# plus-rkwitt/flooder

Measured on AMD Instinct MI355X. Metric: M points×simplices/s (coverage sweep), higher is better.
Workload: dtype f32; 1 GPU; 1M-point 3D Gaussian, 1k landmarks, points_per_edge 30, max_dimension 3, fp32 coverage sweep (BASELINE.json configs[1]); points=1000000, landmarks=1000, top_simplices=6052, top_simplices_rank0=6052, swept_dimension=3, method=cell, parallelism=single GPU

## Files before the change

flooder_amd/_native.py:

```python

from __future__ import annotations

import ctypes
import os
from ctypes import c_char_p, c_float, c_int, c_int32, c_int64, c_uint32, c_void_p

_PKG_DIR = os.path.dirname(os.path.abspath(__file__))
LIB_PATH = os.environ.get("FLOODER_HIP_LIB") or os.path.join(_PKG_DIR, "libflooder_hip.so")



class _Block(ctypes.Structure):

    ABI = 1

    def __init__(self, **fields):
        super().__init__()
        self.size = ctypes.sizeof(self)
        self.abi = self.ABI
        known = {name for name, _ in self._fields_}
        for key, value in fields.items():
            if key not in known:
                raise TypeError(f"{type(self).__name__} has no field {key!r}")
            if value is not None and not isinstance(value, (int, float)):
                value = ptr(value)
            setattr(self, key, value)


def _fields(spec: str):
    kinds = {"p": c_void_p, "i64": c_int64, "i32": c_int32, "u32": c_uint32, "f32": c_float}
    out = []
    for item in spec.replace("\n", " ").split(";"):
        item = item.strip()
        if item:
            kind, name = item.split()
            out.append((name, kinds[kind]))
    return out


class FusedSweep(_Block):

    _fields_ = _fields("""u32 size; u32 abi; p pts_sorted; i64 n_pts; i32 dim; i32 k1; p nodes; p density_grid; p cloud_box;
        p verts; p weights; i32 R; i32 n_faces; i64 n_simplices; p memb; f32 alpha; i32 n_coarse; p coarse_rows; p parents;
        p face_bits; p face_slot; p d2_scratch; p flag_list; p flag_count; p flag_key; p flag_hist; p flag_sorted; p top;
        p top_list; p top_count; p simplex_weight; p plane_scratch; p wit_queue; p wit_item_list; p wit_stats;
        p cell_queue; p defer_list; p defer_c; p defer_ctl; p light_list; p heavy_list; p cell_stats; p finish_ctl;
        p hard_scratch; i32 hard_cap; i32 probed; p finish_stats; p wit_runs; i32 wit_run_len; i32 wit_n_runs;
        i32 planes_ready; i32 reserved; p face_owner; p min_face; p chunk_faces; p tile_faces""")


class SortedSweep(_Block):

    _fields_ = _fields("""u32 size; u32 abi; p pts_sorted; i64 n_pts; i32 dim; i32 k1; p nodes; p verts; p weights; i32 R;
        i32 n_faces; i64 n_simplices; p sample_order; p queue; p memb; p face_bits; p face_slot; p stats; p out_d2;
        i32 shard_rank; i32 shard_world""")


class FpsBatched(_Block):

    _fields_ = _fields("""u32 size; u32 abi; p pts; i64 n_pts; i32 dim; i32 ld; p pts_sorted; p order; i64 start; i32 n_lms;
        i32 reserved; p out_idx; p minsq; p bucket_box; p bucket_keys; p bucket_coord; p work_best; p work_rec; p work_ctr;
        p launches_out""")


class WitnessSearch(_Block):

    _fields_ = _fields("""u32 size; u32 abi; p pts_sorted; i64 n_pts; i32 dim; i32 k1; p nodes; p order; p verts; p weights;
        i32 R; i32 reserved; i64 n_simplices; i64 n_queries; p q_simplex; p q_row; p q_d2; p out_point; p not_found""")


class KnnSweep(_Block):

    _fields_ = _fields("""u32 size; u32 abi; p pts_sorted; i64 n_pts; i32 dim; i32 k1; p nodes; p verts; p weights; i32 R;
        i32 k; i64 n_simplices; i32 stat; i32 reserved; p queue; p out_bits; p stats""")


class KnnSorted(_Block):

    _fields_ = KnnSweep._fields_ + _fields("p sample_order")


# ... 266 lines not shown
```

flooder_amd/core.py:

```python

from __future__ import annotations

import ctypes
import itertools
import math
import os
import weakref
import warnings
from numbers import Integral, Real
from typing import Callable, Dict, List, NamedTuple, Optional, Tuple, Union

import numpy as np
import torch

from . import _native
from .simplex_tree import HAS_GUDHI, SimplexTree, delaunay_cells, delaunay_simplices

__all__ = ["flood_complex", "generate_landmarks", "generate_grid", "generate_uniform_weights",
           "SUPPORTED_DTYPES", "HAS_HIP_KERNELS", "PointIndex", "index_from_host"]

SUPPORTED_DTYPES = (torch.float32, torch.float64)
INF_BITS = 0x7F800000
CAND_ALIGN = 8
SWEEP_CHUNK = 2048
# ... 1488 lines not shown
                or gathered.dim() != 4 or gathered.shape[0] < 1 or tuple(gathered.shape[1:]) != (k, b - a, R)):
            raise ValueError("neighbor_reduce_hook must return every rank's lists as a (W, k, S, R) int32 tensor on the "
                             f"device of the points (W >= 1, (k, S, R) = {(k, b - a, R)}), got "
                             f"{tuple(gathered.shape) if isinstance(gathered, torch.Tensor) else type(gathered).__name__}")
        gathered = gathered.contiguous()
        d2 = torch.empty((b - a, R), dtype=torch.int32, device=dev)
        mrg = _native.KnnMerge(lists=gathered, n_cells=(b - a) * R, n_lists=int(gathered.shape[0]), k=k,
                               stat=NEIGHBOR_STATS.index(stat), out_bits=d2)
        with _span(timer, "merge"):
            _native.check(lib.flooder_knn_merge_f32(ctypes.byref(mrg), st), "flooder_knn_merge_f32")
        _face_epilogue(lib, st, d2, faces, plan.rows_perm, timer=timer, out_face=out_face[a:b])
    return out_face, None


BVH_SORTED_SAMPLES: Optional[bool] = None
SORTED_WORKSPACE_BYTES = 16 << 30
PROFILE_WORKSPACE_BYTES = SORTED_WORKSPACE_BYTES
KNN_MERGE_WORKSPACE_BYTES = PROFILE_WORKSPACE_BYTES
DTM_GRAD_WORKSPACE_BYTES = 4 << 30
SORTED_FUSED_FACES = False
BVH_SORTED_MIN_SAMPLES = 64 * 1024
EMPTY_CACHE_ABOVE_BYTES = 1 << 30
CELL_ALPHA = 1.35
FUSED_FACES = True
CELL_PROBE = True
SHARED_FACE_SLOTS = True
FINISH_HARD_CAP = 32768
CELL_DENSITY_GRID = True
CELL_SUPER = True
WIT_MIN_SIMPLICES = 1536
WIT_MAX_POINTS_PER_SIMPLEX = 400
CELL_WITNESS = True
WIT_RUNS = True
FACE_OWNER = True
FACE_OWNER_GROUPED = False

CTL_FLAG_COUNT, CTL_DEFER, CTL_HIST = 1, 12, 48


def fused_layout(S: int, n_slots: int, wit: bool, owner: bool) -> Tuple[Dict[str, Tuple[int, int]], int]:
    sizes = [("wit_queue", QUEUE_WORDS)] if wit else []
    sizes += [("cell_queue", _native.CELL_QUEUE_WORDS), ("finish_ctl", _native.FINISH_CTL_WORDS), ("top", 2 * S),
              ("ctl", CTL_HIST + _native.FLAG_HIST_WORDS), ("face_bits", n_slots)]
    if owner:
        sizes += [("face_owner", 2 * n_slots), ("result", n_slots)]
    regions, n_words = {}, 0
    for name, words in sizes:
        if name == "face_owner":
            n_words += n_words & 1
        regions[name] = (n_words, words)
        n_words += words
    return regions, n_words


class FusedWorkspace:

    def __init__(self, S: int, R: int, n_faces: int, n_slots: Optional[int], device, wit: bool, owner: bool,
                 planes: Optional[torch.Tensor] = None):
        def empty(shape, dtype=torch.int32):
            return torch.empty(shape, dtype=dtype, device=device)

        regions, self.n_words = fused_layout(S, S * n_faces if n_slots is None else n_slots, wit, owner)
        self.planes = planes if planes is not None else empty(24 * S, torch.float32)
        self.arena = (torch.empty if CELL_SUPER and SWEEP_PREPARE_FUSED else torch.zeros)(self.n_words, dtype=torch.int32,
                                                                                            device=device)
        self.wit_queue = self.face_owner = self.result = None
# ... 45 lines not shown
    w_perm, rows_perm = plan.w_perm, plan.rows_perm

    def sub(a, b):
        return None if stats is None else stats[a:b]

    if S == 0:
        return _no_simplices(faces, R, dev, want_dist)
    if FUSED_FACES and not want_dist and reduce_hook is None and plan.memb_all is not None:
        F = faces.n_faces
        slot_t, n_slots = face_slots if face_slots is not None else (None, None)
        use_wit = (CELL_WITNESS and CELL_SUPER and CELL_PROBE and index.dim in (2, 3) and S >= WIT_MIN_SIMPLICES
                   and index.n <= WIT_MAX_POINTS_PER_SIMPLEX * S and plan.wit is not None)
        use_owner = (FACE_OWNER and face_slots is not None and plan.owner_order and CELL_SUPER and SWEEP_PREPARE_FUSED
                     and plan.sub_faces.numel() == F)
        ws = FusedWorkspace(S, R, F, n_slots, dev, use_wit, use_owner)
        if CELL_SUPER:
            if SWEEP_PREPARE_FUSED:
                _native.check(lib.flooder_simplex_prepare_f32(_native.ptr(index.nodes), index.n, index.dim, _native.ptr(verts),
                                                              k1, S, _native.ptr(ws.wgt), _native.ptr(ws.planes),
                                                              _native.ptr(ws.arena), ws.n_words, st),
                              "flooder_simplex_prepare_f32")
            else:
                _native.check(lib.flooder_simplex_weight_f32(_native.ptr(index.nodes), index.n, index.dim, _native.ptr(verts),
                                                             k1, S, _native.ptr(ws.wgt), st), "flooder_simplex_weight_f32")
        wst = stats[16:40] if use_wit and stats is not None and stats.numel() >= 40 else None
        blk = _native.FusedSweep(
            pts_sorted=index.pts, n_pts=index.n, dim=index.dim, k1=k1, nodes=index.nodes, density_grid=index.dens,
            cloud_box=index.box, verts=verts, weights=w_perm, R=R, n_faces=F, n_simplices=S, memb=plan.memb_all,
            alpha=float(CELL_ALPHA), face_slot=slot_t, cell_stats=sub(0, 9), probed=1 if CELL_PROBE else 0,
            finish_stats=sub(9, 16), **ws.block_fields())
        if use_owner:
            blk.min_face = plan.min_face.data_ptr()
            blk.chunk_faces, blk.tile_faces = plan.chunk_faces.data_ptr(), plan.tile_faces.data_ptr()
        if use_wit:
            blk.n_coarse, blk.coarse_rows, blk.parents = plan.wit[2], plan.wit[0].data_ptr(), plan.wit[1].data_ptr()
            blk.wit_stats = _native.ptr(wst) or None
            if WIT_RUNS and plan.wit_runs is not None:
                blk.wit_runs, blk.wit_run_len, blk.wit_n_runs = plan.wit_runs[0].data_ptr(), plan.wit_runs[1], plan.wit_runs[2]
        blk.planes_ready = 1 if CELL_SUPER and SWEEP_PREPARE_FUSED else 0
        with _span(timer, "sweep"):
            if use_wit:
                _native.check(lib.flooder_fused_witness(ctypes.byref(blk), st), "flooder_fused_witness")
                blk.planes_ready = 1
            _native.check(lib.flooder_fused_cell(ctypes.byref(blk), st), "flooder_fused_cell")
        with _span(timer, "fallback"):
            _native.check(lib.flooder_fused_finish(ctypes.byref(blk), st), "flooder_fused_finish")
        if stats is not None:
            c_d = ws.defer_ctl[:_native.DEFER_CTL_WORDS].tolist()
            LAST_STATS.deferred_chunks = int(c_d[_native.DEFER_CTL_COUNT])
            LAST_STATS.light_heavy = (int(c_d[_native.DEFER_CTL_LIGHT]), int(c_d[_native.DEFER_CTL_HEAVY]))
            LAST_STATS.dense_tiles = int(c_d[_native.DEFER_CTL_TILE_COUNT])
            c_h = ws.finish_ctl[:_native.FINISH_CTL_QUEUES].tolist()
            LAST_STATS.hard_entries = (int(c_h[_native.FINISH_CTL_TOP_HARD_LEN]), int(c_h[_native.FINISH_CTL_REST_HARD_LEN]))
            LAST_STATS.finish_single_left = int(c_h[_native.FINISH_CTL_SINGLE_LEFT])
        if use_owner:
            with _span(timer, "face_max"):
                _native.check(lib.flooder_face_closure_f32(_native.ptr(ws.face_bits), _native.ptr(slot_t),
                                                           _native.ptr(plan.sub_faces), S, F, _native.ptr(ws.result), st),
                              "flooder_face_closure_f32")
            return ws.result, None
        out_face = torch.empty(n_slots if face_slots is not None else (S, F), dtype=torch.float32, device=dev)
        with _span(timer, "face_max"):
            _native.check(lib.flooder_face_values_f32(_native.ptr(ws.face_bits), ws.face_bits.numel(), _native.ptr(out_face), st),
                          "flooder_face_values_f32")
        return out_face, None

# ... 402 lines not shown
```

flooder_amd/csrc/flood_cell.hip:

```cpp

#include <type_traits>

#include "flood_common.hpp"
#include "flood_bvh.hpp"
#include "flood_planes.hpp"

using namespace flooder;

namespace {

constexpr int SPL_CHUNK = 4;
#ifndef FLOODER_CELL_CAPW
#define FLOODER_CELL_CAPW 480
#endif
#ifndef FLOODER_CELL_MAXLEAF
#define FLOODER_CELL_MAXLEAF 584
#endif
#ifndef FLOODER_CELL_WAVES
#define FLOODER_CELL_WAVES 4
#endif
#ifndef FLOODER_CELL_COMPACT
#define FLOODER_CELL_COMPACT 0
#endif
constexpr int CAPW = FLOODER_CELL_CAPW;
// ... 1481 lines not shown
      if (dl.list) {
        if (runs_launch) FLOODER_CELL_LAUNCH(true, SPL_CHUNK, queue);
        FLOODER_CELL_LAUNCH(false, SPL_CHUNK, a.cell_queue + FLOODER_CELL_QUEUE_CHUNKS);
      } else {
        FLOODER_CELL_LAUNCH(false, SPL_CHUNK, queue);
      }
      if (dl.tile_list) FLOODER_CELL_LAUNCH(false, 1, a.cell_queue + FLOODER_CELL_QUEUE_TILES);
#undef FLOODER_CELL_LAUNCH
      return check_launch("cell_sweep");
    } else {
      return fail(FLOODER_E_ARG, "flooder_sweep_cell_f32: only dim 2 and 3");
    }
  }
};

}

namespace flooder {
int launch_simplex_planes(int dim, const float* verts, int k1, int64_t n_simplices, float* tab, hipStream_t st) {
  if (dim == 2)
    hipLaunchKernelGGL((simplex_planes_kernel<2>), dim3((unsigned)((n_simplices + 255) / 256)), dim3(256), 0, st, verts, k1,
                       n_simplices, tab);
  else if (dim == 3)
    hipLaunchKernelGGL((simplex_planes_kernel<3>), dim3((unsigned)((n_simplices + 255) / 256)), dim3(256), 0, st, verts, k1,
                       n_simplices, tab);
  else
    return fail(FLOODER_E_ARG, "simplex planes: only dim 2 and 3");
  return check_launch("simplex_planes");
}
}

namespace {

struct OwnerJob {
  unsigned long long* owner = nullptr;
  const int32_t* slot = nullptr;
  int n_faces = 0;
};
__device__ __forceinline__ void choose_owners(const OwnerJob& oj, const float* __restrict__ weight, int n, int block,
                                              int n_blocks, int tid, int nt) {
  const int64_t total = (int64_t)n * oj.n_faces;
  for (int64_t t = (int64_t)block * nt + tid; t < total; t += (int64_t)n_blocks * nt) {
    const int s = (int)(t / oj.n_faces);
    if (t - (int64_t)s * oj.n_faces == 0) continue;
    atomicMax(&oj.owner[oj.slot[t]], owner_key(s, weight[s]));
  }
}
inline int owner_blocks(const OwnerJob& oj, int n, int nt) {
  if (!oj.owner) return 0;
  const int64_t b = ((int64_t)n * oj.n_faces + 4 * nt - 1) / (4 * nt);
  return (int)(b < 1 ? 1 : (b > 1024 ? 1024 : b));
}

__global__ __launch_bounds__(1024) void split_simplices_kernel(const float* __restrict__ weight, int n, float limit,
                                                               float sparse_limit, int32_t* __restrict__ light,
                                                               int32_t* __restrict__ heavy, int32_t* __restrict__ counts,
                                                               OwnerJob oj) {
  if (blockIdx.x > 0) {
    choose_owners(oj, weight, n, (int)blockIdx.x - 1, (int)gridDim.x - 1, (int)threadIdx.x, 1024);
    return;
  }
  __shared__ int s_cl[16], s_ch[16];
  __shared__ int s_sparse, s_act;
  const int lane = threadIdx.x & 63, wv = threadIdx.x >> 6;
  if (threadIdx.x == 0) { s_sparse = 0; s_act = 0; }
  __syncthreads();
  int mine = 0, act = 0;
  for (int i = threadIdx.x; i < n; i += 1024) {
    const float w = weight[i];
    mine += (w >= 0.f && w <= sparse_limit) ? 1 : 0;
    act += w >= 0.f ? 1 : 0;
  }
#pragma unroll
  for (int o = 32; o > 0; o >>= 1) {
    mine += __shfl_xor(mine, o);
    act += __shfl_xor(act, o);
  }
  if (lane == 0) { atomicAdd(&s_sparse, mine); atomicAdd(&s_act, act); }
  __syncthreads();
  const bool all_heavy = 2 * s_sparse < s_act;
  int n_light = 0, n_heavy = 0;
  for (int base = 0; base < n; base += 1024) {
    const int i = base + threadIdx.x;
    const float w = i < n ? weight[i] : -1.f;
    const bool is_light = w >= 0.f && !all_heavy && w <= limit;
// ... 195 lines not shown
  if (!a.pts_sorted || !a.nodes || !a.verts || !a.plane_scratch || !a.weights || !a.cell_queue || !a.d2_scratch ||
      !a.flag_list || !a.flag_count || a.n_pts < 1 || a.k1 < 1 || a.k1 > FLOODER_MAX_VERTS || a.R < 0 || !(a.alpha > 0.f))
    return fail(FLOODER_E_ARG, who);
  if (a.dim != 2 && a.dim != 3) return fail(FLOODER_E_ARG, "cell sweep: only dim 2 and 3");
  if (a.n_simplices * (int64_t)((a.R + 63) / 64) > 0x7fffffffLL)
    return fail(FLOODER_E_ARG, "cell sweep: too many (simplex, tile) pairs");
  const Levels lv = make_levels(a.n_pts);
  if ((a.n_pts + FLOODER_BVH_LEAF) * (int64_t)(padded_dim(a.dim) * sizeof(float)) >= (1LL << 32) ||
      total_nodes(lv) * (int64_t)(2 * padded_dim(a.dim) * sizeof(float)) >= (1LL << 32))
    return fail(FLOODER_E_ARG, "cell sweep: cloud too large for the cell sweep (use the tree sweep)");
  DensGrid dg;
  if (a.density_grid && a.cloud_box) { dg.grid = a.density_grid; dg.box = a.cloud_box; }
  return dispatch_dim<CellOp>(a.dim, a, lv, acc, dl, dg, (hipStream_t)stream);
}

}

int flooder::fused_cell(const flooder_fused_sweep_t& a, void* stream) {
  if (a.n_simplices == 0 || a.R == 0) return FLOODER_OK;
  if (!a.memb || !a.face_bits || a.n_faces < 1 || a.n_faces > 32 || (a.top && (!a.top_list || !a.top_count)) ||
      (a.defer_list && (!a.defer_c || !a.defer_ctl)) ||
      (a.simplex_weight && (!a.defer_list || !a.light_list || !a.heavy_list)) || (a.flag_key && (!a.flag_hist || !a.top)) ||
      a.n_simplices > 0x7fffffffLL)
    return fail(FLOODER_E_ARG, "flooder_sweep_cell_faces_f32: bad argument");
  const float* const weight = a.simplex_weight;
  int32_t* const light = weight ? a.light_list : nullptr;
  int32_t* const heavy = weight ? a.heavy_list : nullptr;
  int32_t* const split = weight ? a.defer_ctl + FLOODER_DEFER_CTL_LIGHT : nullptr;
  const int n = (int)a.n_simplices;
  const hipStream_t st = (hipStream_t)stream;
  if (a.face_owner && (!weight || !a.face_slot || !a.min_face || !a.chunk_faces || !a.tile_faces))
    return fail(FLOODER_E_ARG, "flooder_fused_cell: face_owner needs simplex_weight, face_slot, min_face, chunk_faces and tile_faces");
  OwnerJob oj;
  if (a.face_owner) { oj.owner = reinterpret_cast<unsigned long long*>(a.face_owner); oj.slot = a.face_slot; oj.n_faces = a.n_faces; }
  if (weight) {
    const bool long_queue = a.n_simplices * (int64_t)((a.R + 255) / 256) >= (int64_t)g_cell_super_min_chunks;
    if (long_queue && (g_cell_split_launches == 2 || a.n_simplices > 7680)) {
      hipLaunchKernelGGL(split_simplices_kernel, dim3(1 + owner_blocks(oj, n, 1024)), dim3(1024), 0, st, weight, n,
                         (float)g_cell_super_weight, (float)g_cell_super_sparse, light, heavy, split, oj);
      if (g_cell_weight_classes)
        hipLaunchKernelGGL(class_order_kernel<SPLIT_THREADS>, dim3(1), dim3(SPLIT_THREADS), 0, st, weight, n,
                           (float)g_cell_super_weight, (float)g_cell_super_sparse, 2, 1, light, heavy, split, OwnerJob{});
    } else if (long_queue) {
      hipLaunchKernelGGL(class_order_kernel<SPLIT_THREADS_LONG>, dim3(1 + owner_blocks(oj, n, SPLIT_THREADS_LONG)),
                         dim3(SPLIT_THREADS_LONG), 0, st, weight, n, (float)g_cell_super_weight, (float)g_cell_super_sparse,
                         (g_cell_weight_classes ? 2 : 0) | 1 | 4, 0, light, heavy, split, oj);
    } else {
      hipLaunchKernelGGL(class_order_kernel<SPLIT_THREADS>, dim3(1 + owner_blocks(oj, n, SPLIT_THREADS)), dim3(SPLIT_THREADS), 0,
                         st, weight, n, (float)g_cell_super_weight, (float)g_cell_super_sparse, g_cell_weight_classes ? 2 : 0,
                         0, light, heavy, split, oj);
    }
  }
  DeferList dl{a.defer_list, a.defer_c, a.defer_list ? a.defer_ctl + FLOODER_DEFER_CTL_COUNT : nullptr, light, heavy,
               split, g_cell_super_n0};
  if (a.defer_list) {
    const int64_t n_chunk_slots = a.n_simplices * (int64_t)((a.R + 255) / 256);
    dl.tile_list = a.defer_list + n_chunk_slots;
    dl.tile_c = a.defer_c + n_chunk_slots;
    dl.tile_count = a.defer_ctl + FLOODER_DEFER_CTL_TILE_COUNT;
  }
  FaceAcc acc{a.memb, a.face_bits, a.n_faces, reinterpret_cast<unsigned long long*>(a.top), a.top_list,
              a.top_count, a.face_slot, a.flag_key, a.flag_hist};
  if (a.face_owner) {
    acc.owner = oj.owner; acc.min_face = a.min_face; acc.chunk_faces = a.chunk_faces; acc.tile_faces = a.tile_faces;
  }
  return sweep_cell_entry(a, acc, dl, "flooder_sweep_cell_faces_f32: bad argument", stream);
}
// ... 70 lines not shown
```

flooder_amd/csrc/flood_common.hpp:

```cpp
#pragma once
#include <hip/hip_runtime.h>
#include <stdint.h>
#include <stdio.h>
#include <string.h>

#include <type_traits>

#include "../../include/flooder_hip.h"

namespace flooder {

constexpr uint32_t INF_BITS = 0x7f800000u;

#define FLOODER_OPTION(name, def, lo, hi, desc) extern int g_##name;
#define FLOODER_OPTION_LIST(name, def, desc, ...) extern int g_##name;
#include "flood_options.def"
#undef FLOODER_OPTION
#undef FLOODER_OPTION_LIST
int launch_simplex_planes(int dim, const float* verts, int k1, int64_t n_simplices, float* tab, hipStream_t st);
char* err_buf();
int fail(int code, const char* msg);
int failf(int code, const char* fmt, ...) __attribute__((format(printf, 2, 3), visibility("hidden")));
int check_launch(const char* what);

// ... 170 lines not shown
struct FaceAcc {
  const uint32_t* memb;
  uint32_t* face_bits;
  int n_faces;
  unsigned long long* top;
  int32_t* top_list;
  int32_t* top_count;
  const int32_t* slot;
  uint32_t* flag_key = nullptr;
  int32_t* flag_hist = nullptr;
  const unsigned long long* owner = nullptr;
  const uint8_t* min_face = nullptr;
  const uint32_t* chunk_faces = nullptr;
  const uint32_t* tile_faces = nullptr;
  __device__ __forceinline__ uint32_t own_mask(int64_t s, int lane) const {
    bool mine = false;
    if (lane > 0 && lane < n_faces) {
      const unsigned long long k =
          __hip_atomic_load(owner + slot[s * (int64_t)n_faces + lane], __ATOMIC_RELAXED, __HIP_MEMORY_SCOPE_AGENT);
      mine = (uint32_t)k == ~(uint32_t)s;
    }
    return (uint32_t)__ballot(mine) | 1u;
  }
  __device__ __forceinline__ int64_t slot_of(int64_t s, int f) const {
    return slot ? (int64_t)slot[s * (int64_t)n_faces + f] : s * (int64_t)n_faces + f;
  }
};

__device__ __forceinline__ unsigned long long owner_key(int s, float w) {
  const uint32_t wb = __float_as_uint(w) < 0x7f800000u ? __float_as_uint(w) : 0x7f800000u;
  const uint32_t hi = w < 0.f ? 0xffffffffu : 0x7fffffffu - wb;
  return ((unsigned long long)hi << 32) | (unsigned long long)(~(uint32_t)s);
}

template <template <int> class F, typename... Args>
int dispatch_dim(int dim, Args&&... args) {
  switch (dim) {
    case 1: return F<1>::run(args...);
    case 2: return F<2>::run(args...);
    case 3: return F<3>::run(args...);
    case 4: return F<4>::run(args...);
    case 5: return F<5>::run(args...);
    case 6: return F<6>::run(args...);
    case 7: return F<7>::run(args...);
    case 8: return F<8>::run(args...);
    default: return fail(FLOODER_E_ARG, "dim must be in 1..8");
  }
}


constexpr int KIND_WORDS = 4;
template <int DIM>
__device__ __forceinline__ void cloud_kind_block(const int32_t* __restrict__ fine, int32_t* __restrict__ kind, int block, int tid,
                                                 int* s_own, int* s_red) {
  constexpr int G = DIM == 2 ? 64 : 16;
  constexpr int GF = 4 * G;
  const int cx = DIM == 3 ? (tid & 15) : (tid & 63);
  const int cy = DIM == 3 ? (tid >> 4) : (4 * block + (tid >> 6));
  const int cz = DIM == 3 ? block : 0;
  const int own_axis = DIM == 3 ? cz : cy;
  int4 r[3][DIM == 3 ? 16 : 4];
#pragma unroll
  for (int d = 0; d < 3; ++d) {
    const int a = own_axis + d - 1;
    const bool ok = a >= 0 && a < G;
    if constexpr (DIM == 3) {
// ... 91 lines not shown
```

flooder_amd/csrc/flood_wit.hip:

```cpp

#include "flood_common.hpp"
#include "flood_bvh.hpp"

using namespace flooder;

namespace {

#ifndef FLOODER_WIT_BLOCKS
#define FLOODER_WIT_BLOCKS 4
#endif
constexpr int WBLOCKS = FLOODER_WIT_BLOCKS;
constexpr int WTHREADS = 256;
constexpr int WWAVES = WTHREADS / 64;
constexpr int WCAP = 960;
constexpr int WLEAF = 1024;
constexpr int WFRONT = 192;
constexpr int WCOARSE = FLOODER_WIT_MAX_COARSE;
constexpr int WFOCUS = 16;
constexpr int WROUNDS = 8;
constexpr int WUR = 256;
constexpr int WQ = 768;
constexpr int WROWS = FLOODER_WIT_MAX_ROWS;
constexpr int UNR = 4;
constexpr int UNRF = 1;
// ... 142 lines not shown
      slo_t[f] = g.slo[f] - tol;
      shi_t[f] = g.shi[f] + tol;
      inv_den[f] = 1.f / (1.001f + g.ps[f]);
      po[f] = g.po[f];
#pragma unroll
      for (int k = 0; k < DIM; ++k) pn[f][k] = g.pn[f][k];
    }
  }
  template <int DP>
  __device__ __forceinline__ float operator()(const float (&x)[DP]) const {
    float e = 0.f;
    float xr[DIM];
#pragma unroll
    for (int k = 0; k < DIM; ++k) {
      e = __builtin_fmaxf(e, __builtin_fmaxf(x[k] - bhi_e[k], blo_e[k] - x[k]));
      xr[k] = x[k] - org[k];
    }
#pragma unroll
    for (int f = 0; f <= DIM; ++f) {
      float dd = -po[f];
#pragma unroll
      for (int k = 0; k < DIM; ++k) dd = __builtin_fmaf(pn[f][k], xr[k], dd);
      e = __builtin_fmaxf(e, __builtin_fmaxf(dd - shi_t[f], slo_t[f] - dd) * inv_den[f]);
    }
    return e;
  }
};

template <int DIM>
__global__ __launch_bounds__(WTHREADS, WBLOCKS) void wit_sweep_kernel(
    const float* __restrict__ pts, const float* __restrict__ nodes, Levels lv, const float* __restrict__ verts,
    const float* __restrict__ plane_tab, const float* __restrict__ weights, int k1, int R, int64_t n_simplices,
    float w_limit, float cmax_mult, float cmax_ext, int min_bins, int flags, int max_open, int max_live, int max_in, int adaptive, int leaf_cap, int max_eval, int sorted_stage, const int32_t* __restrict__ item_list, const int32_t* __restrict__ item_count, WitPlan plan, int32_t* __restrict__ queue, WitOut out, FaceAcc acc,
    unsigned long long* __restrict__ stats) {
  constexpr int DP = padded_dim(DIM);
  __shared__ float4 s_pts[WCAP + 4];
  static_assert(WCAP % SGRP == 0 && SGRP + 4 <= WTHREADS && SGRP % 4 == 0, "whole groups of stage slots, padded by one pass of the workgroup");
  __shared__ int s_leaf[WLEAF];
  __shared__ uint32_t s_qbuf[WQ + WQ / 2];
  __shared__ int s_front[2 * WFRONT];
  __shared__ float s_wit[3 * WCOARSE];
  __shared__ int s_hist[NBIN];
  __shared__ uint32_t s_mf[32];
  __shared__ uint32_t s_unres[WROWS / 32];
  __shared__ uint32_t s_tkey[WROWS / 64];
  __shared__ int s_ftile[WROWS / 64];
  __shared__ int s_gn[MAXL + 2];
  __shared__ int s_ctr[4];
  __shared__ uint16_t s_ur_row[WUR];
  __shared__ uint32_t s_ur_best[WUR];
  __shared__ int16_t s_ur_slot[WUR];
  __shared__ float s_ur_p[WUR * 3];
  __shared__ uint16_t s_focus[WFOCUS];
  __shared__ uint32_t s_fx[8];
  __shared__ float s_rg[Region<DIM>::WORDS];
  __shared__ long long s_item;
  __shared__ int s_off;
  __shared__ float s_run[2];
  __shared__ int s_nrun;
  __shared__ int s_cur[NBIN];
  __shared__ float s_gc[(WCAP + SGRP - 1) / SGRP + 2];
  uint16_t* s_runs = reinterpret_cast<uint16_t*>(s_leaf);
  static_assert(WLEAF * sizeof(int) >= (WROWS / 8) * sizeof(uint16_t), "the run list fits the leaf list (runs of 8 rows or more)");
  uint32_t* s_qub = s_qbuf;
  uint16_t* s_qrow = reinterpret_cast<uint16_t*>(s_qbuf + WQ);
  float4* s_xb = reinterpret_cast<float4*>(s_qbuf);
  constexpr int XB = 256;
  static_assert(XB * sizeof(float4) <= sizeof(uint32_t) * (WQ + WQ / 2) && XB == WTHREADS, "a batch fits the queue's storage");
  const int tid = threadIdx.x;
  const int lane = tid & 63;
  const int wv = tid >> 6;
  const int top = lv.n_levels - 1;
  const int tiles64 = (R + 63) >> 6;
  if (__builtin_amdgcn_readfirstlane(item_count[0]) == 0) return;
  __shared__ unsigned long long s_stat[24];
  enum { ST_HANDLED = 0, ST_HEAVY = 1, ST_OVER = 2, ST_DENSE = 3, ST_STAGED = 4, ST_CCERT = 5, ST_LIVE = 6, ST_ROUNDS = 7,
// ... 241 lines not shown
        v.x = x[u][0];
        v.y = x[u][1];
        v.z = DIM > 2 ? x[u][DIM > 2 ? 2 : 0] : 0.f;
        v.w = 0.f;
        if (sorted_stage) {
          if (keep) {
            const int pos = atomicAdd(&s_cur[(int)eb], 1);
            if (pos < WCAP) s_pts[pos] = v;
          }
          continue;
        }
        const unsigned long long m = __ballot(keep);
        if (m != 0ull) {
          int base = 0;
          if (lane == 0) base = atomicAdd(&s_ctr[0], __popcll(m));
          base = wave_uniform(base);
          if (keep) s_pts[base + lane_rank(m)] = v;
        }
      }
    }
    }
    __syncthreads();
    const int K = sorted_stage ? n_stage : s_ctr[0];
    if (K + tid < ((K + SGRP - 1) & ~(SGRP - 1)) + 4) s_pts[K + tid] = make_float4(__builtin_inff(), __builtin_inff(), __builtin_inff(), 0.f);
    if (sorted_stage && wv == 0) {
      const int end = lane < n_keep_bins ? s_cur[lane] : 0x7fffffff;
      int bin = 0;
      for (int g = 0; g * SGRP < K; ++g) {
        const int b = __popcll(__ballot(end <= g * SGRP));
        if (lane == g) bin = b;
      }
      if (lane * SGRP < K) s_gc[lane] = bin > 0 ? (float)bin / bin_scale : -__builtin_inff();
    }
    if (tid < acc.n_faces)
      s_mf[tid] = __hip_atomic_load(acc.face_bits + acc.slot_of(s, tid), __ATOMIC_RELAXED, __HIP_MEMORY_SCOPE_AGENT);
    __syncthreads();
    if (tid == 0) { count(ST_STAGED, (unsigned long long)K); count(ST_BINS, (unsigned long long)n_keep_bins); }
    WPHASE(3);

    auto make_sample = [&](int r, float (&p)[DIM]) {
#pragma unroll
      for (int k = 0; k < DIM; ++k) p[k] = 0.f;
      if (k1 == 4) {
        const float4 w4 = *reinterpret_cast<const float4*>(weights + (int64_t)r * 4);
        const float wj[4] = {w4.x, w4.y, w4.z, w4.w};
#pragma unroll
        for (int j = 0; j < 4; ++j) {
#pragma unroll
          for (int k = 0; k < DIM; ++k) p[k] = __builtin_fmaf(wj[j], vs[j * DIM + k], p[k]);
        }
      } else {
        for (int j = 0; j < k1; ++j) {
          const float w = weights[(int64_t)r * k1 + j];
#pragma unroll
          for (int k = 0; k < DIM; ++k) p[k] = __builtin_fmaf(w, vs[j * DIM + k], p[k]);
        }
      }
    };
    auto deliver = [&](bool on, uint32_t mb, float val) {
      uint32_t um = wave_or_u32(on ? mb : 0u);
      while (um) {
        const int f = __builtin_ctz(um);
        um &= um - 1u;
        const uint32_t v = wave_max_u32((on && ((mb >> f) & 1u)) ? __float_as_uint(val) : 0u);
        if (lane == 0 && v > s_mf[f]) {
          atomicMax(&acc.face_bits[acc.slot_of(s, f)], v);
          atomicMax(&s_mf[f], v);
        }
      }
// ... 310 lines not shown
          dg2 = __builtin_fminf(dg2, d2);
        }
        const float t = __builtin_sqrtf(dg2) + __builtin_fmaf(__uint_as_float(rb.z), sigma, a_abs);
        float bnd = (t * t) * 1.000004f;
        if (bnd < 1e-30f) bnd = __builtin_inff();
        const uint32_t thr = threshold(valid ? rb.x : 0u);
        const bool keep = valid && !(__float_as_uint(bnd) <= thr);
        const unsigned long long m = __ballot(keep);
        if (m != 0ull) {
          int base = 0;
          if (lane == 0) base = atomicAdd(&s_nrun, __popcll(m));
          base = wave_uniform(base);
          if (keep) s_runs[base + lane_rank(m)] = (uint16_t)i;
        }
        if (stats) { const unsigned long long md = __ballot(valid && !keep); if (lane == 0) count(ST_RUNS, (unsigned long long)__popcll(md)); }
      }
      __syncthreads();
      n_run_rows = s_nrun << run_shift;
      tail0 = plan.n_runs << run_shift;
    }
    const int n_fine = n_run_rows + (R - tail0);
    auto load_rows = [&](int g0, FineRows& fr) {
#pragma unroll
      for (int u = 0; u < UNRF; ++u) {
        const int idx = g0 + u * WTHREADS + tid;
        fr.valid[u] = idx < n_fine;
        const int r = !fr.valid[u] ? R - 1
                      : idx < n_run_rows ? ((int)s_runs[idx >> run_shift] << run_shift) + (idx & ((1 << run_shift) - 1))
                                         : tail0 + (idx - n_run_rows);
        fr.rr[u] = r;
        if (k1 == 4) fr.w4[u] = *reinterpret_cast<const float4*>(weights + (int64_t)fr.rr[u] * 4);
        fr.par[u] = plan.parents[fr.rr[u]];
        fr.mb[u] = fr.valid[u] ? acc.memb[fr.rr[u]] : 0u;
      }
    };
    FineRows ring[FDEPTH];
#pragma unroll
    for (int a = 0; a < FDEPTH; ++a)
      if (a * WTHREADS * UNRF < n_fine) load_rows(a * WTHREADS * UNRF, ring[a]);
    for (int g0 = 0; g0 < n_fine; g0 += WTHREADS * UNRF) {
      const FineRows cur = ring[0];
#pragma unroll
      for (int a = 0; a + 1 < FDEPTH; ++a) ring[a] = ring[a + 1];
      if (g0 + FDEPTH * WTHREADS * UNRF < n_fine) load_rows(g0 + FDEPTH * WTHREADS * UNRF, ring[FDEPTH - 1]);
#pragma unroll
      for (int u = 0; u < UNRF; ++u) {
        if (g0 + u * WTHREADS >= n_fine) break;
        float p[DIM];
        if (k1 == 4) {
          const float wj[4] = {cur.w4[u].x, cur.w4[u].y, cur.w4[u].z, cur.w4[u].w};
#pragma unroll
          for (int k = 0; k < DIM; ++k) p[k] = 0.f;
#pragma unroll
          for (int j = 0; j < 4; ++j) {
#pragma unroll
            for (int k = 0; k < DIM; ++k) p[k] = __builtin_fmaf(wj[j], vs[j * DIM + k], p[k]);
          }
        } else {
          make_sample(cur.rr[u], p);
        }
        float ub = __builtin_inff();
#pragma unroll
        for (int j = 0; j < 4; ++j) {
          const int c = (int)((cur.par[u] >> (8 * j)) & 0xffu);
          float t0 = p[0] - s_wit[3 * c + 0];
          float d2 = t0 * t0;
// ... 162 lines not shown
          }
          if (lane == 0) count(ST_FLAGGED, (unsigned long long)n_ft);
        }
        for (int i = wv; i < n_ft; i += WWAVES) {
          const int r = s_ftile[i] * 64 + lane;
          if (r < R && !((s_unres[r >> 5] >> (r & 31)) & 1u)) out.d2[s * (int64_t)R + r] = SETTLED_BIT;
        }
      }
    }
    WIT_REC(10, 1); WIT_REC(11, __builtin_amdgcn_s_memrealtime() - t_item0); WIT_REC(7, s_ctr[2]);
    if (tid == 0) { out.weight[s] = -1.f; if ((s & 7) == 0) atomicAdd(&queue[8], 1); }
    if (tid == 0) count(ST_HANDLED, 1);
    WPHASE(7);
  }
  __syncthreads();
  if (stats) {
#ifdef FLOODER_WIT_TIMERS
    if (tid == 0)
      for (int i = 0; i < 10; ++i) atomicAdd(&stats[12 + i], t_ph[i]);
#endif
#ifdef FLOODER_WIT_TIMERS
    const bool flush = tid < 12 || tid >= 22;
#else
    const bool flush = tid < 12 || tid >= ST_RUNS;
#endif
    if (tid < 24 && flush && s_stat[tid] != 0ull) atomicAdd(&stats[tid], s_stat[tid]);
  }
}

constexpr int WCLASSES = 4;
constexpr int WLIST_LDS = 8192;
__global__ __launch_bounds__(1024) void wit_list_kernel(const float* __restrict__ weight, int n, float limit,
                                                        int32_t* __restrict__ list, int32_t* __restrict__ count,
                                                        const int32_t* __restrict__ kind, int surface_pct) {
  __shared__ int s_cnt[WCLASSES][16];
  __shared__ float s_w[WLIST_LDS];
  const int lane = threadIdx.x & 63, wv = threadIdx.x >> 6;
  if (kind != nullptr) {
    const int inner = kind[2], all = kind[3];
    if (all > 0 && (long long)inner * 100 < (long long)all * surface_pct) {
      if (threadIdx.x == 0) count[0] = 0;
      return;
    }
  }
  auto cls = [&](float w) -> int {
    if (!(w >= 0.f) || !(w <= limit)) return -1;
    return w > 0.5f * limit ? 0 : (w > 0.25f * limit ? 1 : (w > 0.125f * limit ? 2 : 3));
  };
  const bool staged = n <= WLIST_LDS;
  if (staged) {
#pragma unroll
    for (int u = 0; u < WLIST_LDS / 1024; ++u) {
      const int i = u * 1024 + (int)threadIdx.x;
      if (i < n) s_w[i] = weight[i];
    }
    __syncthreads();
  }
  const int per = ((n + 1023) / 1024) | 1;
  const int i0 = (int)threadIdx.x * per < n ? (int)threadIdx.x * per : n;
  const int i1 = i0 + per < n ? i0 + per : n;
  int cnt[WCLASSES];
#pragma unroll
  for (int k = 0; k < WCLASSES; ++k) cnt[k] = 0;
  for (int i = i0; i < i1; ++i) {
    const int c = cls(staged ? s_w[i] : weight[i]);
#pragma unroll
    for (int k = 0; k < WCLASSES; ++k) cnt[k] += c == k ? 1 : 0;
  }
  int excl[WCLASSES];
#pragma unroll
  for (int k = 0; k < WCLASSES; ++k) {
    int v = cnt[k];
#pragma unroll
    for (int o = 1; o < 64; o <<= 1) {
      const int t = __shfl_up(v, o);
      v += lane >= o ? t : 0;
// ... 64 lines not shown
    }
  }
  for (int64_t i = pt_off[s] + tid; i < pt_off[s + 1]; i += 64) {
    float x[DIM];
#pragma unroll
    for (int k = 0; k < DIM; ++k) x[k] = pts[i * DIM + k];
    const float e = excess(x);
    const float eb = e * bin_scale;
    pt_excess[i] = e;
    pt_bin[i] = eb < (float)NBIN ? (int)eb : NBIN;
  }
  for (int r = tid; r < R; r += 64) {
    float p[DIM];
#pragma unroll
    for (int k = 0; k < DIM; ++k) p[k] = 0.f;
    for (int j = 0; j < k1; ++j) {
      const float w = weights[(int64_t)r * k1 + j];
#pragma unroll
      for (int k = 0; k < DIM; ++k) p[k] = __builtin_fmaf(w, vs[j * DIM + k], p[k]);
    }
    const float dl = rg.slack(p);
    float* o = samples + (s * R + r) * (int64_t)(DIM + 1);
#pragma unroll
    for (int k = 0; k < DIM; ++k) o[k] = p[k];
    o[DIM] = dl;
    float* l = limits + (s * R + r) * (int64_t)(NBIN + 1);
    for (int k = 0; k <= NBIN; ++k) l[k] = Region<DIM>::limit(dl, (float)k / bin_scale);
  }
}

template <int DIM>
struct WitOp {
  static int run(const flooder_fused_sweep_t& a, const Levels& lv, WitPlan plan, WitOut out, FaceAcc acc,
                 const int32_t* kind, hipStream_t st) {
    if constexpr (DIM == 2 || DIM == 3) {
      const int64_t ns = a.n_simplices;
      int32_t* item_count = a.wit_queue + FLOODER_WIT_QUEUE_ITEM_COUNT;
      if (!a.planes_ready) {
        const int rc = launch_simplex_planes(DIM, a.verts, a.k1, ns, a.plane_scratch, st);
        if (rc != FLOODER_OK) return rc;
      }
      hipLaunchKernelGGL(wit_list_kernel, dim3(1), dim3(1024), 0, st, out.weight, (int)ns, (float)g_wit_weight, a.wit_item_list,
                         item_count, g_wit_surface_pct > 0 ? kind : nullptr, g_wit_surface_pct);
      const int grid = (int)(ns < g_wit_grid ? ns : g_wit_grid);
      const int R = a.R;
      hipLaunchKernelGGL((wit_sweep_kernel<DIM>), dim3(grid), dim3(WTHREADS), 0, st, a.pts_sorted, a.nodes, lv, a.verts, a.plane_scratch, a.weights, a.k1,
                         R, ns, (float)g_wit_weight, 0.01f * (float)g_wit_cmax_pct, 0.01f * (float)g_wit_cmax_ext_pct, g_wit_min_bins, g_wit_flags, g_wit_max_open, (int)((int64_t)R * g_wit_max_live_pct / 100), (int)((int64_t)R * g_wit_max_in_pct / 100), g_wit_adaptive, g_wit_max_leaves < WLEAF ? g_wit_max_leaves : WLEAF, g_wit_max_eval, g_wit_sorted_stage, a.wit_item_list, item_count, plan, a.wit_queue, out, acc,
                         reinterpret_cast<unsigned long long*>(a.wit_stats));
      return check_launch("wit_sweep");
    } else {
      return fail(FLOODER_E_ARG, "flooder_sweep_witness_f32: only dim 2 and 3");
    }
  }
};

}

int flooder::fused_witness(const flooder_fused_sweep_t& a, void* stream) {
  if (a.n_simplices == 0 || a.R == 0) return FLOODER_OK;
  if (!a.pts_sorted || !a.nodes || !a.verts || !a.weights || !a.coarse_rows || !a.parents || !a.wit_queue || !a.d2_scratch ||
      !a.memb || !a.face_bits || !a.flag_list || !a.flag_count || !a.simplex_weight || !a.wit_item_list || !a.plane_scratch ||
      a.n_pts < 1 || a.k1 < 1 || a.k1 > FLOODER_MAX_VERTS || a.R < 1 || a.R > WROWS || a.n_coarse < 1 || a.n_coarse > WCOARSE ||
      a.n_faces < 1 || a.n_faces > 32 || (a.top && (!a.top_list || !a.top_count)) || (a.flag_key && !a.flag_hist) ||
      a.n_simplices > 0x7fffffffLL)
    return fail(FLOODER_E_ARG, "flooder_sweep_witness_f32: bad argument");
  if (a.dim != 2 && a.dim != 3) return fail(FLOODER_E_ARG, "flooder_sweep_witness_f32: only dim 2 and 3");
  if (a.n_simplices * (int64_t)((a.R + 63) / 64) > 0x7fffffffLL)
    return fail(FLOODER_E_ARG, "flooder_sweep_witness_f32: too many (simplex, tile) pairs");
  const Levels lv = make_levels(a.n_pts);
  if ((a.n_pts + FLOODER_BVH_LEAF) * (int64_t)(padded_dim(a.dim) * sizeof(float)) >= (1LL << 32) ||
      total_nodes(lv) * (int64_t)(2 * padded_dim(a.dim) * sizeof(float)) >= (1LL << 32))
    return fail(FLOODER_E_ARG, "flooder_sweep_witness_f32: cloud too large");
  const bool have_runs = a.wit_runs && a.wit_n_runs > 0;
  int run_shift = 0;
  if (have_runs) {
    const int run_len = a.wit_run_len;
    if (run_len < 8 || run_len > a.R || (run_len & (run_len - 1)) != 0 || (int64_t)a.wit_n_runs * run_len > a.R || a.k1 > 4)
      return fail(FLOODER_E_ARG, "flooder_fused_witness: bad run table");
    while ((1 << run_shift) < run_len) ++run_shift;
  }
  const bool use_runs = have_runs && g_wit_runs != 0;
  return dispatch_dim<WitOp>(
      a.dim, a, lv,
      WitPlan{a.coarse_rows, a.parents, a.n_coarse, use_runs ? reinterpret_cast<const uint4*>(a.wit_runs) : nullptr,
              run_shift, use_runs ? a.wit_n_runs : 0},
      WitOut{a.d2_scratch, a.flag_list, a.flag_count, a.simplex_weight},
      FaceAcc{a.memb, a.face_bits, a.n_faces, reinterpret_cast<unsigned long long*>(a.top), a.top_list, a.top_count,
              a.face_slot, a.flag_key, a.flag_hist},
      a.density_grid ? a.density_grid + (flooder_density_grid_words(a.dim) - KIND_WORDS) : nullptr, (hipStream_t)stream);
}

extern "C" {

int flooder_wit_max_rows(void) { return WROWS; }
int flooder_wit_max_coarse(void) { return WCOARSE; }

int flooder_sweep_witness_f32(const float* pts_sorted, int64_t n_pts, int dim, const float* nodes, const float* verts,
                              const float* weights, int k1, int R, int64_t n_simplices, const int32_t* coarse_rows,
                              int n_coarse, const uint32_t* parents, int32_t* queue, uint32_t* d2_scratch,
                              const uint32_t* memb, int n_faces, uint32_t* face_bits, const int32_t* face_slot,
                              int32_t* flag_list, int32_t* flag_count, uint32_t* flag_key, int32_t* flag_hist,
                              uint64_t* top, int32_t* top_list, int32_t* top_count, float* simplex_weight,
                              int32_t* item_list, float* plane_scratch, uint64_t* stats, void* stream) {
  flooder_fused_sweep_t a{};
  a.pts_sorted = pts_sorted; a.n_pts = n_pts; a.dim = dim; a.nodes = nodes; a.verts = verts; a.weights = weights;
  a.k1 = k1; a.R = R; a.n_simplices = n_simplices; a.coarse_rows = coarse_rows; a.n_coarse = n_coarse;
  a.parents = parents; a.wit_queue = queue; a.d2_scratch = d2_scratch; a.memb = memb; a.n_faces = n_faces;
  a.face_bits = face_bits; a.face_slot = face_slot; a.flag_list = flag_list; a.flag_count = flag_count;
  a.flag_key = flag_key; a.flag_hist = flag_hist; a.top = top; a.top_list = top_list; a.top_count = top_count;
  a.simplex_weight = simplex_weight; a.wit_item_list = item_list; a.plane_scratch = plane_scratch; a.wit_stats = stats;
  return fused_witness(a, stream);
}

int flooder_wit_probe_f32(const float* verts, int dim, int64_t n_simplices, float cmax_frac, const float* pts,
                          const int64_t* pt_off, int64_t n_points, const float* weights, int R, float* out, int32_t* bins,
                          void* stream) {
  if (!verts || !pts || !pt_off || !weights || !out || !bins || n_simplices < 1 || n_simplices > 0x7fffffffLL ||
      n_points < 0 || R < 1 || !(cmax_frac > 0.f) || (dim != 2 && dim != 3))
    return fail(FLOODER_E_ARG, "flooder_wit_probe_f32: bad argument");
  hipStream_t st = (hipStream_t)stream;
  const int64_t S = n_simplices;
  const int W = dim == 2 ? Region<2>::WORDS : Region<3>::WORDS, E = 2 * dim + 3 * (dim + 1), C = 2 + 2 * dim;
// ... 20 lines not shown
```

include/flooder_hip.h:

```cpp
#ifndef FLOODER_HIP_H
#define FLOODER_HIP_H

#include <stdint.h>

#ifdef __cplusplus
extern "C" {
#endif

#define FLOODER_ABI_VERSION 1

#define FLOODER_OK 0
#define FLOODER_E_ARG (-1)
#define FLOODER_E_LAUNCH (-2)
#define FLOODER_E_DEVICE (-3)

#define FLOODER_MAX_DIM 8
#define FLOODER_MAX_VERTS 9
#define FLOODER_CAND_ALIGN 8
#define FLOODER_SWEEP_CHUNK 2048
#define FLOODER_TILE_SAMPLES 512
#define FLOODER_BVH_LEAF 16
#define FLOODER_BVH_FANOUT 64
#define FLOODER_BVH_MAX_LEVELS 6
#define FLOODER_QUEUE_SHARDS 16
// ... 240 lines not shown
  int32_t* flag_count;
  uint32_t* flag_key;
  int32_t* flag_hist;
  int32_t* flag_sorted;
  uint64_t* top;
  int32_t* top_list;
  int32_t* top_count;
  float* simplex_weight;
  float* plane_scratch;
  int32_t* wit_queue;
  int32_t* wit_item_list;
  uint64_t* wit_stats;
  int32_t* cell_queue;
  int32_t* defer_list;
  float* defer_c;
  int32_t* defer_ctl;
  int32_t* light_list;
  int32_t* heavy_list;
  uint64_t* cell_stats;
  int32_t* finish_ctl;
  uint64_t* hard_scratch;
  int32_t hard_cap;
  int32_t probed;
  uint64_t* finish_stats;
  const uint32_t* wit_runs;
  int32_t wit_run_len;
  int32_t wit_n_runs;
  int32_t planes_ready;
  int32_t reserved;
  uint64_t* face_owner;
  const uint8_t* min_face;
  const uint32_t* chunk_faces;
  const uint32_t* tile_faces;
} flooder_fused_sweep_t;

int flooder_fused_witness(const flooder_fused_sweep_t* p, void* stream);
int flooder_fused_cell(const flooder_fused_sweep_t* p, void* stream);
int flooder_fused_finish(const flooder_fused_sweep_t* p, void* stream);

typedef struct flooder_sorted_sweep_s {
  uint32_t size, abi;
  const float* pts_sorted;
  int64_t n_pts;
  int32_t dim;
  int32_t k1;
  const float* nodes;
  const float* verts;
  const float* weights;
  int32_t R;
  int32_t n_faces;
  int64_t n_simplices;
  const int32_t* sample_order;
  int32_t* queue;
  const uint32_t* memb;
  uint32_t* face_bits;
  const int32_t* face_slot;
  uint64_t* stats;
  uint32_t* out_d2;
  int32_t shard_rank;
  int32_t shard_world;
} flooder_sorted_sweep_t;
int flooder_sorted_faces(const flooder_sorted_sweep_t* p, void* stream);
int flooder_sorted_minima(const flooder_sorted_sweep_t* p, void* stream);

typedef struct flooder_fps_batched_s {
  uint32_t size, abi;
// ... 225 lines not shown
```

Before: 6.658 million M points×simplices/s.

## Assign face owners before the witness sweep and skip non-owned face updates

Extra workgroups in the witness list kernel pre-assign an owning simplex to each shared face using a tagged atomicMax key over in-range simplex weights. The witness sweep then loads these owners plus a subface closure of face bits. It masks membership for rows whose minimal face is not owned by the current simplex, so duplicate face accumulation across neighbouring simplices is skipped. This adds an ownership pass, extra per-simplex loads and shuffles, and a change to cell-stage owner selection. It relies on `sub_faces` being supplied by the plan.

```diff
diff --git a/flooder_amd/_native.py b/flooder_amd/_native.py
--- a/flooder_amd/_native.py
+++ b/flooder_amd/_native.py
@@ -46,7 +46,7 @@
         p top_list; p top_count; p simplex_weight; p plane_scratch; p wit_queue; p wit_item_list; p wit_stats;
         p cell_queue; p defer_list; p defer_c; p defer_ctl; p light_list; p heavy_list; p cell_stats; p finish_ctl;
         p hard_scratch; i32 hard_cap; i32 probed; p finish_stats; p wit_runs; i32 wit_run_len; i32 wit_n_runs;
-        i32 planes_ready; i32 reserved; p face_owner; p min_face; p chunk_faces; p tile_faces""")
+        i32 planes_ready; i32 reserved; p face_owner; p min_face; p chunk_faces; p tile_faces; p sub_faces""")
 
 
 class SortedSweep(_Block):
diff --git a/flooder_amd/core.py b/flooder_amd/core.py
--- a/flooder_amd/core.py
+++ b/flooder_amd/core.py
@@ -1544,6 +1544,7 @@
 WIT_MAX_POINTS_PER_SIMPLEX = 400
 CELL_WITNESS = True
 WIT_RUNS = True
+WIT_OWNER = True
 FACE_OWNER = True
 FACE_OWNER_GROUPED = False
 
@@ -1655,6 +1656,8 @@
         if use_owner:
             blk.min_face = plan.min_face.data_ptr()
             blk.chunk_faces, blk.tile_faces = plan.chunk_faces.data_ptr(), plan.tile_faces.data_ptr()
+            if WIT_OWNER:
+                blk.sub_faces = plan.sub_faces.data_ptr()
         if use_wit:
             blk.n_coarse, blk.coarse_rows, blk.parents = plan.wit[2], plan.wit[0].data_ptr(), plan.wit[1].data_ptr()
             blk.wit_stats = _native.ptr(wst) or None
diff --git a/flooder_amd/csrc/flood_cell.hip b/flooder_amd/csrc/flood_cell.hip
--- a/flooder_amd/csrc/flood_cell.hip
+++ b/flooder_amd/csrc/flood_cell.hip
@@ -1537,25 +1537,6 @@
 
 namespace {
 
-struct OwnerJob {
-  unsigned long long* owner = nullptr;
-  const int32_t* slot = nullptr;
-  int n_faces = 0;
-};
-__device__ __forceinline__ void choose_owners(const OwnerJob& oj, const float* __restrict__ weight, int n, int block,
-                                              int n_blocks, int tid, int nt) {
-  const int64_t total = (int64_t)n * oj.n_faces;
-  for (int64_t t = (int64_t)block * nt + tid; t < total; t += (int64_t)n_blocks * nt) {
-    const int s = (int)(t / oj.n_faces);
-    if (t - (int64_t)s * oj.n_faces == 0) continue;
-    atomicMax(&oj.owner[oj.slot[t]], owner_key(s, weight[s]));
-  }
-}
-inline int owner_blocks(const OwnerJob& oj, int n, int nt) {
-  if (!oj.owner) return 0;
-  const int64_t b = ((int64_t)n * oj.n_faces + 4 * nt - 1) / (4 * nt);
-  return (int)(b < 1 ? 1 : (b > 1024 ? 1024 : b));
-}
 
 __global__ __launch_bounds__(1024) void split_simplices_kernel(const float* __restrict__ weight, int n, float limit,
                                                                float sparse_limit, int32_t* __restrict__ light,
@@ -1817,7 +1798,10 @@
   if (a.face_owner && (!weight || !a.face_slot || !a.min_face || !a.chunk_faces || !a.tile_faces))
     return fail(FLOODER_E_ARG, "flooder_fused_cell: face_owner needs simplex_weight, face_slot, min_face, chunk_faces and tile_faces");
   OwnerJob oj;
-  if (a.face_owner) { oj.owner = reinterpret_cast<unsigned long long*>(a.face_owner); oj.slot = a.face_slot; oj.n_faces = a.n_faces; }
+  if (a.face_owner) {
+    oj.owner = reinterpret_cast<unsigned long long*>(a.face_owner); oj.slot = a.face_slot; oj.n_faces = a.n_faces;
+    oj.pre = wit_owner_on(a) ? 1 : 0;
+  }
   if (weight) {
     const bool long_queue = a.n_simplices * (int64_t)((a.R + 255) / 256) >= (int64_t)g_cell_super_min_chunks;
     if (long_queue && (g_cell_split_launches == 2 || a.n_simplices > 7680)) {
diff --git a/flooder_amd/csrc/flood_common.hpp b/flooder_amd/csrc/flood_common.hpp
--- a/flooder_amd/csrc/flood_common.hpp
+++ b/flooder_amd/csrc/flood_common.hpp
@@ -226,6 +226,50 @@
   const uint32_t hi = w < 0.f ? 0xffffffffu : 0x7fffffffu - wb;
   return ((unsigned long long)hi << 32) | (unsigned long long)(~(uint32_t)s);
 }
+__device__ __forceinline__ unsigned long long pre_owner_key(int s, float w) {
+  return owner_key(s, w) | 0x8000000000000000ull;
+}
+
+struct OwnerJob {
+  unsigned long long* owner = nullptr;
+  const int32_t* slot = nullptr;
+  int n_faces = 0;
+  int pre = 0;
+};
+__device__ __forceinline__ void choose_owners(const OwnerJob& oj, const float* __restrict__ weight, int n, int block,
+                                              int n_blocks, int tid, int nt) {
+  const int64_t total = (int64_t)n * oj.n_faces;
+  for (int64_t t = (int64_t)block * nt + tid; t < total; t += (int64_t)n_blocks * nt) {
+    const int s = (int)(t / oj.n_faces);
+    if (t - (int64_t)s * oj.n_faces == 0) continue;
+    const float w = weight[s];
+    if (oj.pre && w < 0.f) continue;
+    atomicMax(&oj.owner[oj.slot[t]], owner_key(s, w));
+  }
+}
+__device__ __forceinline__ void choose_pre_owners(const OwnerJob& oj, const float* __restrict__ weight, float limit, int n,
+                                                  int block, int n_blocks, int tid, int nt) {
+  const int64_t total = (int64_t)n * oj.n_faces;
+  for (int64_t t = (int64_t)block * nt + tid; t < total; t += (int64_t)n_blocks * nt) {
+    const int s = (int)(t / oj.n_faces);
+    if (t - (int64_t)s * oj.n_faces == 0) continue;
+    const float w = weight[s];
+    if (!(w >= 0.f) || !(w <= limit)) continue;
+    atomicMax(&oj.owner[oj.slot[t]], pre_owner_key(s, w));
+  }
+}
+inline int owner_blocks(const OwnerJob& oj, int n, int nt) {
+  if (!oj.owner) return 0;
+  const int64_t b = ((int64_t)n * oj.n_faces + 4 * nt - 1) / (4 * nt);
+  return (int)(b < 1 ? 1 : (b > 1024 ? 1024 : b));
+}
+
+#ifndef FLOODER_WIT_OWNER
+#define FLOODER_WIT_OWNER 1
+#endif
+inline bool wit_owner_on(const flooder_fused_sweep_t& a) {
+  return FLOODER_WIT_OWNER != 0 && a.face_owner && a.min_face && a.sub_faces && a.face_slot;
+}
 
 template <template <int> class F, typename... Args>
 int dispatch_dim(int dim, Args&&... args) {
diff --git a/flooder_amd/csrc/flood_wit.hip b/flooder_amd/csrc/flood_wit.hip
--- a/flooder_amd/csrc/flood_wit.hip
+++ b/flooder_amd/csrc/flood_wit.hip
@@ -198,7 +198,7 @@
     const float* __restrict__ pts, const float* __restrict__ nodes, Levels lv, const float* __restrict__ verts,
     const float* __restrict__ plane_tab, const float* __restrict__ weights, int k1, int R, int64_t n_simplices,
     float w_limit, float cmax_mult, float cmax_ext, int min_bins, int flags, int max_open, int max_live, int max_in, int adaptive, int leaf_cap, int max_eval, int sorted_stage, const int32_t* __restrict__ item_list, const int32_t* __restrict__ item_count, WitPlan plan, int32_t* __restrict__ queue, WitOut out, FaceAcc acc,
-    unsigned long long* __restrict__ stats) {
+    const uint32_t* __restrict__ sub_faces, unsigned long long* __restrict__ stats) {
   constexpr int DP = padded_dim(DIM);
   __shared__ float4 s_pts[WCAP + 4];
   static_assert(WCAP % SGRP == 0 && SGRP + 4 <= WTHREADS && SGRP % 4 == 0, "whole groups of stage slots, padded by one pass of the workgroup");
@@ -208,6 +208,7 @@
   __shared__ float s_wit[3 * WCOARSE];
   __shared__ int s_hist[NBIN];
   __shared__ uint32_t s_mf[32];
+  __shared__ uint32_t s_own;
   __shared__ uint32_t s_unres[WROWS / 32];
   __shared__ uint32_t s_tkey[WROWS / 64];
   __shared__ int s_ftile[WROWS / 64];
@@ -515,9 +516,28 @@
       }
       if (lane * SGRP < K) s_gc[lane] = bin > 0 ? (float)bin / bin_scale : -__builtin_inff();
     }
-    if (tid < acc.n_faces)
-      s_mf[tid] = __hip_atomic_load(acc.face_bits + acc.slot_of(s, tid), __ATOMIC_RELAXED, __HIP_MEMORY_SCOPE_AGENT);
+    if (sub_faces == nullptr) {
+      if (tid < acc.n_faces)
+        s_mf[tid] = __hip_atomic_load(acc.face_bits + acc.slot_of(s, tid), __ATOMIC_RELAXED, __HIP_MEMORY_SCOPE_AGENT);
+      if (tid == 0) s_own = 0xffffffffu;
+    } else if (wv == 1) {
+      const bool on = lane < acc.n_faces;
+      const int64_t sl = on ? (int64_t)acc.slot[s * (int64_t)acc.n_faces + lane] : 0;
+      const uint32_t raw = on ? __hip_atomic_load(acc.face_bits + sl, __ATOMIC_RELAXED, __HIP_MEMORY_SCOPE_AGENT) : 0u;
+      const unsigned long long key =
+          on && lane > 0 ? __hip_atomic_load(acc.owner + sl, __ATOMIC_RELAXED, __HIP_MEMORY_SCOPE_AGENT) : 0ull;
+      const uint32_t sub = on ? sub_faces[lane] : 0u;
+      uint32_t closed = raw;
+      for (int g = 0; g < acc.n_faces; ++g) {
+        const uint32_t v = (uint32_t)__shfl((int)raw, g);
+        closed = ((sub >> g) & 1u) && v > closed ? v : closed;
+      }
+      if (on) s_mf[lane] = closed;
+      const uint32_t mine = (uint32_t)__ballot(on && lane > 0 && (uint32_t)key == ~(uint32_t)s) | 1u;
+      if (lane == 0) s_own = mine;
+    }
     __syncthreads();
+    const uint32_t own = (uint32_t)__builtin_amdgcn_readfirstlane((int)s_own);
     if (tid == 0) { count(ST_STAGED, (unsigned long long)K); count(ST_BINS, (unsigned long long)n_keep_bins); }
     WPHASE(3);
 
@@ -894,6 +914,7 @@
         if (k1 == 4) fr.w4[u] = *reinterpret_cast<const float4*>(weights + (int64_t)fr.rr[u] * 4);
         fr.par[u] = plan.parents[fr.rr[u]];
         fr.mb[u] = fr.valid[u] ? acc.memb[fr.rr[u]] : 0u;
+        if (acc.min_face && !((own >> acc.min_face[fr.rr[u]]) & 1u)) fr.mb[u] = 0u;
       }
     };
     FineRows ring[FDEPTH];
@@ -1122,16 +1143,20 @@
 constexpr int WLIST_LDS = 8192;
 __global__ __launch_bounds__(1024) void wit_list_kernel(const float* __restrict__ weight, int n, float limit,
                                                         int32_t* __restrict__ list, int32_t* __restrict__ count,
-                                                        const int32_t* __restrict__ kind, int surface_pct) {
+                                                        const int32_t* __restrict__ kind, int surface_pct, OwnerJob oj) {
   __shared__ int s_cnt[WCLASSES][16];
   __shared__ float s_w[WLIST_LDS];
   const int lane = threadIdx.x & 63, wv = threadIdx.x >> 6;
   if (kind != nullptr) {
     const int inner = kind[2], all = kind[3];
     if (all > 0 && (long long)inner * 100 < (long long)all * surface_pct) {
-      if (threadIdx.x == 0) count[0] = 0;
+      if (blockIdx.x == 0 && threadIdx.x == 0) count[0] = 0;
       return;
     }
+  }
+  if (blockIdx.x > 0) {
+    choose_pre_owners(oj, weight, limit, n, (int)blockIdx.x - 1, (int)gridDim.x - 1, (int)threadIdx.x, 1024);
+    return;
   }
   auto cls = [&](float w) -> int {
     if (!(w >= 0.f) || !(w <= limit)) return -1;
@@ -1262,7 +1287,7 @@
 template <int DIM>
 struct WitOp {
   static int run(const flooder_fused_sweep_t& a, const Levels& lv, WitPlan plan, WitOut out, FaceAcc acc,
-                 const int32_t* kind, hipStream_t st) {
+                 const int32_t* kind, const uint32_t* sub_faces, hipStream_t st) {
     if constexpr (DIM == 2 || DIM == 3) {
       const int64_t ns = a.n_simplices;
       int32_t* item_count = a.wit_queue + FLOODER_WIT_QUEUE_ITEM_COUNT;
@@ -1270,12 +1295,15 @@
         const int rc = launch_simplex_planes(DIM, a.verts, a.k1, ns, a.plane_scratch, st);
         if (rc != FLOODER_OK) return rc;
       }
-      hipLaunchKernelGGL(wit_list_kernel, dim3(1), dim3(1024), 0, st, out.weight, (int)ns, (float)g_wit_weight, a.wit_item_list,
-                         item_count, g_wit_surface_pct > 0 ? kind : nullptr, g_wit_surface_pct);
+      OwnerJob oj;
+      if (acc.owner) { oj.owner = const_cast<unsigned long long*>(acc.owner); oj.slot = acc.slot; oj.n_faces = acc.n_faces; oj.pre = 1; }
+      hipLaunchKernelGGL(wit_list_kernel, dim3(1 + owner_blocks(oj, (int)ns, 1024)), dim3(1024), 0, st, out.weight, (int)ns,
+                         (float)g_wit_weight, a.wit_item_list, item_count, g_wit_surface_pct > 0 ? kind : nullptr,
+                         g_wit_surface_pct, oj);
       const int grid = (int)(ns < g_wit_grid ? ns : g_wit_grid);
       const int R = a.R;
       hipLaunchKernelGGL((wit_sweep_kernel<DIM>), dim3(grid), dim3(WTHREADS), 0, st, a.pts_sorted, a.nodes, lv, a.verts, a.plane_scratch, a.weights, a.k1,
-                         R, ns, (float)g_wit_weight, 0.01f * (float)g_wit_cmax_pct, 0.01f * (float)g_wit_cmax_ext_pct, g_wit_min_bins, g_wit_flags, g_wit_max_open, (int)((int64_t)R * g_wit_max_live_pct / 100), (int)((int64_t)R * g_wit_max_in_pct / 100), g_wit_adaptive, g_wit_max_leaves < WLEAF ? g_wit_max_leaves : WLEAF, g_wit_max_eval, g_wit_sorted_stage, a.wit_item_list, item_count, plan, a.wit_queue, out, acc,
+                         R, ns, (float)g_wit_weight, 0.01f * (float)g_wit_cmax_pct, 0.01f * (float)g_wit_cmax_ext_pct, g_wit_min_bins, g_wit_flags, g_wit_max_open, (int)((int64_t)R * g_wit_max_live_pct / 100), (int)((int64_t)R * g_wit_max_in_pct / 100), g_wit_adaptive, g_wit_max_leaves < WLEAF ? g_wit_max_leaves : WLEAF, g_wit_max_eval, g_wit_sorted_stage, a.wit_item_list, item_count, plan, a.wit_queue, out, acc, sub_faces,
                          reinterpret_cast<unsigned long long*>(a.wit_stats));
       return check_launch("wit_sweep");
     } else {
@@ -1310,14 +1338,17 @@
     while ((1 << run_shift) < run_len) ++run_shift;
   }
   const bool use_runs = have_runs && g_wit_runs != 0;
+  FaceAcc acc{a.memb, a.face_bits, a.n_faces, reinterpret_cast<unsigned long long*>(a.top), a.top_list, a.top_count,
+              a.face_slot, a.flag_key, a.flag_hist};
+  const bool own = wit_owner_on(a);
+  if (own) { acc.owner = reinterpret_cast<const unsigned long long*>(a.face_owner); acc.min_face = a.min_face; }
   return dispatch_dim<WitOp>(
       a.dim, a, lv,
       WitPlan{a.coarse_rows, a.parents, a.n_coarse, use_runs ? reinterpret_cast<const uint4*>(a.wit_runs) : nullptr,
               run_shift, use_runs ? a.wit_n_runs : 0},
-      WitOut{a.d2_scratch, a.flag_list, a.flag_count, a.simplex_weight},
-      FaceAcc{a.memb, a.face_bits, a.n_faces, reinterpret_cast<unsigned long long*>(a.top), a.top_list, a.top_count,
-              a.face_slot, a.flag_key, a.flag_hist},
-      a.density_grid ? a.density_grid + (flooder_density_grid_words(a.dim) - KIND_WORDS) : nullptr, (hipStream_t)stream);
+      WitOut{a.d2_scratch, a.flag_list, a.flag_count, a.simplex_weight}, acc,
+      a.density_grid ? a.density_grid + (flooder_density_grid_words(a.dim) - KIND_WORDS) : nullptr,
+      own ? a.sub_faces : nullptr, (hipStream_t)stream);
 }
 
 extern "C" {
diff --git a/include/flooder_hip.h b/include/flooder_hip.h
--- a/include/flooder_hip.h
+++ b/include/flooder_hip.h
@@ -296,6 +296,7 @@
   const uint8_t* min_face;
   const uint32_t* chunk_faces;
   const uint32_t* tile_faces;
+  const uint32_t* sub_faces;
 } flooder_fused_sweep_t;
 
 int flooder_fused_witness(const flooder_fused_sweep_t* p, void* stream);
```

Result: no change. 6.709 million M points×simplices/s (median of 6 runs) (+0.8%).
